# yyNoBug/VAE_segmentation

Measured on AMD Instinct MI355X. Metric: 3D train-step volumes/sec at 96^3 batch=2 (joint VAE+seg), higher is better.
Workload: dtype bf16; 1 GPU; configs[1]: 96^3 joint VAE+seg training step (joint_train), batch=2/GPU, bf16 activations + fp32 accumulate, SGD momentum 0.9, VAE frozen, HIP-graph replay; global_batch=2, parallelism=dp1, activation_recomputation=False, tail_in_graph=True, nranks=1, grad_exchange=none (1 rank)

## Files before the change

include/vaeseg.h:

```cpp
#ifndef VAESEG_H
#define VAESEG_H
#include <stddef.h>
#include <stdint.h>

#ifdef __cplusplus
extern "C" {
#endif

#define VS_VERSION 500

enum { VS_F32 = 0, VS_BF16 = 1, VS_F16 = 2, VS_F32X3 = 3  };
#ifndef VS_STAT_SLOTS
#define VS_STAT_SLOTS 4
#endif
enum { VS_OK = 0, VS_EINVAL = -1, VS_ESHAPE = -2, VS_EDTYPE = -3, VS_EWORKSPACE = -4, VS_EALIGN = -5 };

enum {
    VS_CONV_K3 = 0,
    VS_CONV_K2S2 = 1,
    VS_CONV_T2S2 = 2,
    VS_WGRAD_SLABS = 16,
    VS_CONV_UP = 3
};

enum {
    VS_PACK_ROWS_D0 = 0,
    VS_PACK_ROWS_D1_FLIP = 1,
    VS_PACK_SCATTER_D1 = 2
};

int vs_version(void);
int vs_stat_slots(void);
int vs_stat_interleaved(void);
const char* vs_strerror(int code);
int vs_get_deterministic(void);

int vs_up_supported(int cin, int cm, int co, int dtype);
int vs_up_compose_sizes(int cin, int cm, int co, size_t* out6);
int vs_up_compose(const float* w2, const float* b2, const float* w3, float* weff, void* img_fwd, void* img_bwd, int* taps_fwd, int* taps_bwd,
                  float* btab, int cin, int cm, int co, int dtype, void* stream);
int vs_up_conv_fwd(const void* x, const double* x_stats, const void* img_fwd, const int* taps_fwd, const float* btab, void* y, double* y_stats,
                   int n, int d, int h, int w, int cin, int co, int dtype, float eps, void* stream);
int vs_up_faces(const void* gy, double* G, int n, int fd, int fh, int fw, int co, int dtype, void* stream);
int vs_up_chain(const float* dweff27, const double* G, const float* w2, const float* b2, const float* w3, float* dw2, float* db2, float* dw3,
                int cin, int cm, int co, void* stream);
int vs_up_conv_bwd_data(const void* gy, const void* img_bwd, const int* taps_bwd, void* gx, const void* mask_x, const double* mask_stats,
                        double* sums, int n, int d, int h, int w, int co, int cin, int dtype, float eps, void* stream);

size_t vs_packed_weight_bytes(int rows, int c_pad, int ntaps, int dtype);
int vs_pack_weight(const float* src, void* dst, int d0, int d1, int ntaps, int c_pad, int form, int dtype, void* stream);

typedef struct vs_pack_desc {
    const float* src;
    void* dst;
    int d0, d1, ntaps, c_pad, form, dtype;
    int first_block;
    int pad_;
    long long total;
} vs_pack_desc;
int vs_pack_weight_multi(const vs_pack_desc* descs, int n_desc, int total_blocks, void* stream);

int vs_conv_gather_fwd(const void* x, const double* x_stats, const void* w_packed, const float* bias,
                       void* y, double* y_stats, int n, int d, int h, int w, int c_in, int m_out,
                       int kind, int dtype, float eps, void* stream);

int vs_conv_scatter_fwd(const void* x, const double* x_stats, const void* w_packed, const float* bias,
                        void* y, int n, int d, int h, int w, int c_in, int m_out, int dtype, float eps, void* stream);

int vs_conv_gather_bwd_data(const void* x, const void* w_packed, void* y, const void* mask_x, const double* mask_stats,
                            double* sums, int n, int d, int h, int w, int c_in, int m_out, int kind, int dtype, float eps,
                            void* stream);
int vs_conv_scatter_bwd_data(const void* x, const void* w_packed, void* y, const void* mask_x, const double* mask_stats,
                             double* sums, int n, int d, int h, int w, int c_in, int m_out, int dtype, float eps, void* stream);
int vs_conv_k3_fused_apply_supported(int n, int d, int h, int w, int c_in, int m_out, int lazy_input, int dtype);
int vs_conv_k3_bwd_data_wgrad_supported(int n, int d, int h, int w, int c_in, int m_out, int dtype);
int vs_conv_k3_bwd_data_wgrad_slabs(int n, int d, int h, int w);
int vs_conv_k3_bwd_data_wgrad(const void* g, const void* act_x, const double* act_stats, const double* act_sums, const void* w_packed, void* y,
                              const void* mask_x, const double* mask_stats, double* sums, float* slabs, int n, int d, int h, int w, int c_in,
                              int m_out, int dtype, float eps, void* stream);
int vs_conv_k3_softmax2_bwd_data(const float* prob, const float* gprob, const void* gprob_cl, const void* w_packed, void* y, const void* mask_x,
                                 const double* mask_stats, double* sums, float* slabs, double* bias_part, int n, int d, int h, int w, int dtype,
                                 float eps, float drop_p, unsigned long long drop_seed, void* stream);
typedef struct vs_config {
    int k3_small;
    int k3_tall;
    int k3_wgs_per_cu;
    int k3t_wgs_per_cu;
    int k3f_min_wgs;
    int mt_min_wgs;
    int f32_limbs;
    int g1_limbs;
    int k3x_ck;
    int k3x_toeplitz;
    int fuse_wgrad;
    int epilogue_apply;
    int chain;
    int k2s2_stream;
    int k2s8_wgs_per_cu;
    int up_wgs_per_cu;
    int up_rb;
    int wgrad_uber;
    int wgrad_mpack;
    int wgrad_swap;
    int wgrad_big;
    int wgrad_xcd;
    int k3_short_tiles;
    int wgrad_bias_fold;
    int hist_form;
    long long wgrad_wgs;
    long long wgrad_f32_tiles;
    long long wgrad_group_wgs;
    long long wgrad_big_min_voxels;
} vs_config;
int vs_config_bytes(void);
int vs_config_from_env(vs_config* c);
int vs_get_config(vs_config* out);
int vs_set_config(const vs_config* cfg);
int vs_conv_k3_bwd_data_applied_supported(int n, int d, int h, int w, int c_in, int m_out, int dtype);
int vs_conv_k3_bwd_data_applied(const void* x, const void* w_packed, void* y, const void* mask_x, const double* mask_stats, double* sums,
                                unsigned int* sync, unsigned int* fault, int n, int d, int h, int w, int c_in, int m_out, int dtype, float eps, void* stream);
int vs_conv_s2_bwd_data_applied_supported(int n, int d, int h, int w, int c_in, int m_out, int scatter, int dtype);
int vs_conv_s2_bwd_data_applied(const void* x, const void* w_packed, void* y, const void* mask_x, const double* mask_stats, double* sums, const void* add,
                                unsigned int* sync, unsigned int* fault, int n, int d, int h, int w, int c_in, int m_out, int scatter, int dtype, float eps,
                                void* stream);
typedef struct vs_chain_layer {
    const void* x;
    const double* x_stats;
    const void* w_packed;
    void* y;
    double* y_stats;
    const void* mask_x;
    const double* mask_stats;
    double* sums;
    int c_in, m_out;
    int apply;
    int reserved_;
} vs_chain_layer;
int vs_conv_k3_chain_supported(int n, int d, int h, int w, int c_max, int dtype);
long long vs_conv_k3_chain_sync_bytes(int n);
int vs_conv_k3_chain(const vs_chain_layer* layers, int n_layers, int backward, const void* add, unsigned int* sync, unsigned int* fault,
                     int n, int d, int h, int w, int dtype, float eps, void* stream);
int vs_conv_k3_f32_limbs(int d, int h, int w, int c_in);

int vs_conv_k3_bwd_data_fused_apply(const void* g, const void* act_x, const double* act_stats, const double* act_sums,
                                    const void* w_packed, void* y, const void* mask_x, const double* mask_stats, double* sums,
                                    void* dx_out, int n, int d, int h, int w, int c_in, int m_out, int dtype, float eps, void* stream);

int vs_conv_k3_softmax2_fwd(const void* x, const double* x_stats, const void* w_packed, const float* bias,
                            float* prob, int n, int d, int h, int w, int c_in, int dtype, float eps, void* stream);
int vs_conv_k3_softmax2_dropout_fwd(const void* x, const double* x_stats, const void* w_packed, const float* bias,
                                    float* prob, int n, int d, int h, int w, int c_in, int dtype, float eps, float drop_p,
                                    unsigned long long drop_seed, void* stream);
int vs_conv_k3_softmax2_cl_fwd(const void* x, const double* x_stats, const void* w_packed, const float* bias,
                               float* prob, void* prob_cl, int n, int d, int h, int w, int c_in, int dtype, float eps, float drop_p,
                               unsigned long long drop_seed, void* stream);

size_t vs_conv_wgrad_workspace_bytes(int n, int dp, int hp, int wp, int m_ch, int c_ch, int kind);
int vs_conv_wgrad(const void* p, const double* p_stats, const void* q, const double* q_stats, float* dw,
                  void* workspace, size_t workspace_bytes, int n, int dp, int hp, int wp, int m_ch, int c_ch,
                  int m_real, int c_real, int kind, int dtype, float eps, void* stream);
typedef struct vs_wgrad_desc {
    const void* p; const double* p_stats;
    const void* q; const double* q_stats;
    float* dw;
    const void* bias_g; float* db;
// ... 266 lines not shown
```

vae_segmentation_amd/modules.py:

```python
import torch
import torch.nn as nn

from . import ops

_DEFAULT_DTYPE = torch.float32


def set_default_kernel_dtype(dtype):
    global _DEFAULT_DTYPE
    if dtype not in ops.KERNEL_DTYPES:
        raise TypeError("kernel dtype must be torch.float32, torch.bfloat16 or torch.float16")
    _DEFAULT_DTYPE = dtype


def set_kernel_dtype(module, dtype):
    if dtype not in ops.KERNEL_DTYPES:
        raise TypeError("kernel dtype must be torch.float32, torch.bfloat16 or torch.float16")
    for m in module.modules():
        if hasattr(m, "kernel_dtype"):
            m.kernel_dtype = dtype
    return module


class Act:
# ... 220 lines not shown
        self.top_ch = f[5]
        flat = f[5] * self.side ** 3
        self.fc_mean = nn.Linear(flat, dim)
        self.fc_std = nn.Linear(flat, dim)
        self.fc2 = nn.Linear(dim, flat)
        self.up1 = Up(f[5], f[4], norm_type=norm_type, soft=False)
        self.up2 = Up(f[4], f[3], norm_type=norm_type, soft=False)
        self.up3 = Up(f[3], f[2], norm_type=norm_type, soft=False)
        self.up4 = Up(f[2], f[1], norm_type=norm_type, soft=False)
        self.up5 = Up(f[1], f[0], norm_type=norm_type, soft=False)
        self.out_block = nn.Conv3d(f[0], n_class, 3, padding=1)
        self.final = nn.Softmax(dim=1)
        self.n_class = n_class
        self.spatial = spatial
        self.kernel_dtype = _DEFAULT_DTYPE

    def forward(self, x, if_random=False, scale=1, mid_input=False, dropout=0.0, noise=None):
        ops._require_cuda(x)
        if not mid_input:
            if x.shape[-1] != self.spatial:
                raise ValueError("VAE built for spatial=%d got input side %d" % (self.spatial, x.shape[-1]))
            ops.stats_arena_begin(x.device)
            a = Act(ops.planar_input(x, self.kernel_dtype), None)
            a = self.in_block(a)
            if a.stats is not None:
                ops.mark_defer_apply(a.raw, self.in_block.conv[0])
            for blk in (self.down1, self.down2, self.down3, self.down4, self.down5):
                a = _run_block(blk, a)
                if blk is not self.down5 and a.stats is not None:
                    ops.mark_defer_apply(a.raw, blk.conv[1].conv[6])
            feat = ops.Materialize.apply(a.raw, a.stats, None, None)
            x_mean, x_std = ops.LinearCLPair.apply(feat, self.fc_mean.weight, self.fc_mean.bias, False,
                                                   self.fc_std.weight, self.fc_std.bias, True)
            if if_random and isinstance(noise, ops.LatentStream):
                z, _ = ops.ReparamPhilox.apply(x_mean, x_std, noise, scale)
            elif if_random:
                if noise is None:
                    noise = torch.randn(x_mean.shape, device=x_mean.device, dtype=torch.float32)
                z = ops.Reparam.apply(x_mean, x_std, noise.to(x_mean.device, torch.float32).contiguous(), scale)
            else:
                z = x_mean
        else:
            ops.stats_arena_begin(x.device)
            z = x
        h = ops.LinearToCL.apply(z, self.fc2.weight, self.fc2.bias, self.top_ch, self.side, self.kernel_dtype)
        a = Act(h, None)
        for blk in (self.up1, self.up2, self.up3, self.up4, self.up5):
            a = _dropout(_run_block(blk, a), dropout)
            if a.stats is not None:
                ops.mark_defer_apply(a.raw, blk.conv[1].conv[6])
        recon = ops.ConvK3Softmax.apply(a.raw, a.stats, self.out_block.weight, self.out_block.bias)
        if not mid_input:
            return recon, x_mean, x_std
        return recon


class Segmentation(nn.Module):

    def __init__(self, n_channels, n_class, norm_type=2, n_fmaps=[8, 16, 32, 64, 128, 256]):
        super().__init__()
        _check_n_class(n_class)
        f = list(n_fmaps)
        self.in_block = Conv(n_channels, f[0], norm_type=norm_type, soft=False)
        self.down1 = Down(f[0], f[1], norm_type=norm_type, soft=False)
        self.down2 = Down(f[1], f[2], norm_type=norm_type, soft=False)
        self.down3 = Down(f[2], f[3], norm_type=norm_type, soft=False)
        self.down4 = Down(f[3], f[4], norm_type=norm_type, soft=False)
        self.up2 = Up(f[4], f[3], norm_type=norm_type, soft=False)
        self.up3 = Up(f[3], f[2], norm_type=norm_type, soft=False)
        self.up4 = Up(f[2], f[1], norm_type=norm_type, soft=False)
        self.up5 = Up(f[1], f[0], norm_type=norm_type, soft=False)
        self.out_block = nn.Conv3d(f[0], n_class, 3, padding=1)
        self.final = nn.Softmax(dim=1)
        self.n_class = n_class
        self.kernel_dtype = _DEFAULT_DTYPE

    def forward(self, data_dict, in_key, out_key, dropout=0.0):
        x = data_dict[in_key]
        ops._require_cuda(x)
        if any(s % 16 for s in x.shape[2:]):
            raise ValueError("Segmentation needs spatial sizes that are multiples of 16, got %s" % (tuple(x.shape[2:]),))
        ops.stats_arena_begin(x.device)
        a = Act(ops.PackPlanar.apply(x, self.kernel_dtype), None)
        x1 = self.in_block(a)
        x2 = _run_block(self.down1, x1)
        x3 = _run_block(self.down2, x2)
        x4 = _run_block(self.down3, x3)
        x5 = _run_block(self.down4, x4)
        u = _dropout(_run_block(self.up2, x5), dropout)
        u = _run_block(self.up3, u)
        u = _dropout(Act(ops.Materialize.apply(u.raw, u.stats, x3.raw, x3.stats, True), None), dropout)
        tap4 = u.raw
        u = _run_block(self.up4, u)
        u = _dropout(Act(ops.Materialize.apply(u.raw, u.stats, x2.raw, x2.stats, True), None), dropout)
        if getattr(self, "ds_taps", False):
            data_dict["ds_feats"] = [u.raw, tap4]
        u = _dropout(_run_block(self.up5, u), dropout)
        if u.stats is not None:
            ops.mark_defer_apply(u.raw, self.up5.conv[1].conv[6])
        if dropout:
            data_dict[out_key] = ops.out_block_softmax(u.raw, u.stats, self.out_block.weight, self.out_block.bias,
                                                       float(dropout), ops.next_dropout_seed())
        else:
            data_dict[out_key] = ops.out_block_softmax(u.raw, u.stats, self.out_block.weight, self.out_block.bias)
        return data_dict


class DeepSupervision(nn.Module):

    def __init__(self, seg, levels=2):
        super().__init__()
        levels = int(levels)
        if levels not in (1, 2):
            raise ValueError("DeepSupervision: 1 or 2 levels (the half- and quarter-resolution skip sums), got %r" % (levels,))
        chans = [seg.up5.conv[0].in_channels, seg.up4.conv[0].in_channels][:levels]
        for c in chans:
            if c not in ops.DS_CHANNELS:
                raise NotImplementedError("DeepSupervision: the fused head reads %s feature channels, got %d" % ("/".join(map(str, ops.DS_CHANNELS)), c))
        self.heads = nn.ModuleList([nn.Conv3d(c, seg.n_class, 1) for c in chans])
        seg.ds_taps = True

    def forward(self, batch, target, scales=None, **loss_args):
        feats = batch.get("ds_feats")
        if feats is None:
            raise RuntimeError("DeepSupervision: the batch holds no 'ds_feats' — was it produced by the Segmentation this module was built on?")
        scales = [1.0] * len(self.heads) if scales is None else list(scales)
        if len(scales) != len(self.heads):
            raise ValueError("DeepSupervision: %d scales for %d levels" % (len(scales), len(self.heads)))
        return [ops.ds_head(feats[i], head.weight, head.bias, target, 2 << i, scale=scales[i], **loss_args) for i, head in enumerate(self.heads)]


class Joint(nn.Module):

    def __init__(self, models, vae_forward_scale=0.0, vae_decoder_dropout=0.0, seg_dropout=0.0):
        super().__init__()
        self.Seg = models[0]
        self.Vae = models[1]
        self.vae_forward_scale = vae_forward_scale
        self.vae_decoder_dropout = vae_decoder_dropout
        self.seg_dropout = seg_dropout

    def forward(self, data_dict, in_key, out_key, out_key_recon, dropout=False):
        with ops.arena_scope(data_dict[in_key].device):
            if dropout:
                data_dict = self.Seg(data_dict, in_key, out_key, dropout=self.seg_dropout)
                data_dict[out_key_recon], _, _ = self.Vae(data_dict[out_key], if_random=False, scale=self.vae_forward_scale,
                                                          dropout=self.vae_decoder_dropout)
            else:
                data_dict = self.Seg(data_dict, in_key, out_key)
                data_dict[out_key_recon], data_dict["mean"], data_dict["std"] = self.Vae(
                    data_dict[out_key], if_random=False, scale=self.vae_forward_scale)
        return data_dict


def _linear(x2d, fc, relu):
    return ops.LinearCL.apply(x2d.contiguous().view(x2d.shape[0], 1, 1, 1, x2d.shape[1]), fc.weight, fc.bias, relu)


class Encoder(nn.Module):

    def __init__(self, n_channels, dim, norm_type=2, n_fmaps=[8, 16, 32, 64, 128, 256], soft=False, spatial=128):
        super().__init__()
        if spatial % 32 or spatial < 64:
            raise ValueError("spatial must be a multiple of 32 and >= 64")
        f = list(n_fmaps)
        self.in_block = Conv(n_channels, f[0], norm_type=norm_type, soft=False)
        self.down1 = Down(f[0], f[1], norm_type=norm_type, soft=False)
# ... 113 lines not shown
```

vae_segmentation_amd/ops.py:

```python
import collections as _collections
import contextlib as _contextlib
import ctypes as _ctypes
import os
import weakref as _weakref

import torch

from . import _lib
from ._lib import (VS_BF16, VS_CONV_K2S2, VS_CONV_K3, VS_CONV_UP, VS_F16, VS_F32, VS_PACK_ROWS_D0, VS_PACK_ROWS_D1_FLIP,
                   VS_PACK_SCATTER_D1, _contig, _p, _require_cuda, _stream, check, lib)
from .volume import *
from .volume import signed_distance
from .volume import (PATCH_CHUNK, PATCH_LABEL_DTYPES, PATCH_MAX_CLASSES, PATCH_MAX_SOURCES, patch_gather, patch_index,
                     patch_pick)

_DT_TORCH = {VS_F32: torch.float32, VS_BF16: torch.bfloat16, VS_F16: torch.float16}
_DT_VS = {v: k for k, v in _DT_TORCH.items()}
KERNEL_DTYPES = tuple(_DT_VS)
VS_F32X3 = 3
F32X3 = "f32x3"
_DT_TORCH[VS_F32X3] = F32X3
_DT_VS[F32X3] = VS_F32X3
_F32_LIMBS = bool(lib.vs_conv_k3_f32_limbs(96, 96, 96, 8))

# ... 711 lines not shown
    _GROUP["enabled"] = bool(enabled)


def wgrad_grouping():
    return _GROUP["enabled"]


def set_wgrad_split(first=None):
    flush_wgrads()
    _GROUP["split"] = first


def drop_stale_wgrads():
    g = _GROUP
    if g["descs"] and not _PENDING["queued"]:
        return
    g["descs"], g["keep"] = [], []
    _PENDING.reset()


def _queue_desc(weight, d, dtype, nb, fl, voxels, keep):
    g = _GROUP
    if g["descs"] and g["dtype"] != dtype:
        flush_wgrads()
    g["dtype"] = dtype
    first = g["split"] is None or bool(g["split"](weight))
    g["descs"].append((d, first, nb, fl, voxels))
    g["keep"].extend(t for t in keep if t is not None)
    if not _PENDING.join():
        flush_wgrads()


def _group_submit(weight, keep, wgrad_args, bias_args, gw, gb, up_co=0):
    p, ps, q, qs, m_real, c_real, kind = wgrad_args
    n, dp, hp, wp_, m_ch = p.shape
    gw_ptr = gw if isinstance(gw, int) else gw.data_ptr()
    if kind == VS_CONV_UP:
        dp, hp, wp_, m_ch = dp // 2, hp // 2, wp_ // 2, 8 * up_co
    d = WgradDesc(p.data_ptr(), _p(ps), q.data_ptr(), _p(qs), gw_ptr, None, None, 0, 0, 0,
                  n, dp, hp, wp_, m_ch, q.shape[-1], m_real, c_real, kind, up_co)
    if bias_args is not None:
        bg = bias_args[0]
        gb_ptr = gb if isinstance(gb, int) else gb.data_ptr()
        d.bias_g, d.db, d.bias_rows, d.bias_c_ch, d.bias_c_real = bg.data_ptr(), gb_ptr, bg.numel() // bg.shape[-1], bg.shape[-1], bias_args[1]
        keep = tuple(keep) + (bg,)
    taps = 8 if kind == VS_CONV_K2S2 else 27
    nb = (p.numel() + q.numel() // q.shape[-1] * c_real) * _esize(p) + m_real * c_real * taps * 4 if kind == VS_CONV_UP else \
        (p.numel() // m_ch * m_real + q.numel() // q.shape[-1] * c_real) * _esize(p) + m_real * c_real * taps * 4
    fl = 2.0 * (q.numel() // q.shape[-1]) * taps * m_real * c_real if kind == VS_CONV_UP else 2.0 * (p.numel() // m_ch) * taps * m_real * c_real
    _queue_desc(weight, d, p.dtype, nb, fl, n * dp * hp * wp_, keep)


def pending_wgrads():
    return len(_GROUP["descs"])


def flush_wgrads(first_only=False):
    g = _GROUP
    if not g["descs"]:
        return
    now = [e for e in g["descs"] if e[1]] if first_only else g["descs"]
    later = [e for e in g["descs"] if not e[1]] if first_only else []
    g["descs"] = later
    if not now:
        return
    _issue_wgrads(now)
    if not later:
        _run_up_jobs()
        g["keep"] = []


FUSE_WGRAD = os.environ.get("VS_FUSE_WGRAD", "1") != "0"
VS_WGRAD_SLABS = 16


def _count_use(weight):
    u = getattr(weight, "_vs_use", None)
    if u is None or u[0] != _PENDING["epoch"]:
        weight._vs_use = [_PENDING["epoch"], 1]
    else:
        u[1] += 1


def _wgrad_fusable(gy, x, weight):
    if not (FUSE_WGRAD and _GROUP["enabled"] and gy.dtype != torch.float32 and gy.shape[-1] == 8 and x.shape[-1] == 8):
        return False
    if getattr(weight, "_vs_use", None) != [_PENDING["epoch"], 1] or id(weight) in _PENDING["slots"]:
        return False
    if not (weight.is_leaf and weight.grad is None and not _has_hooks(weight) and not torch.is_grad_enabled()):
        return False
    n, d, h, w, _ = gy.shape
    return bool(lib.vs_conv_k3_bwd_data_wgrad_supported(n, d, h, w, 8, 8, vs_dtype(gy)))


def _group_submit_slabs(weight, slabs, nslabs, m_real, c_real, keep, bias=None):
    gw = _grad_slot(weight, weight.shape)
    gb = None
    d = WgradDesc(slabs.data_ptr(), None, None, None, gw.data_ptr(), None, None, 0, 0, 0, nslabs, 0, 0, 0, 8, 8, m_real, c_real, VS_WGRAD_SLABS, 0)
    if bias is not None:
        gb = _grad_slot(bias[0], (m_real,))
        d.bias_g, d.db, d.bias_rows, d.bias_c_ch, d.bias_c_real = bias[1].data_ptr(), gb.data_ptr(), nslabs, m_real, m_real
    _PENDING["slots"][id(weight)] = _Slot(gw.data_ptr(), _p(gb), True)
    _queue_desc(weight, d, keep[0].dtype, float(slabs.numel() * 4), 0.0, 0, (None if bias is None else bias[1], slabs))
    return gw, gb


def _grad_slot(param, shape):
    view = getattr(param, "_vs_grad_view", None)
    if view is not None and param.grad is None:
        return view.detach()
    return torch.empty(shape, dtype=torch.float32, device=param.device)


def _has_hooks(t):
    return bool(getattr(t, "_backward_hooks", None)) or bool(getattr(t, "_post_accumulate_grad_hooks", None))


def _side_grads(weight, keep, wgrad_args, bias_args, bias=None):
    grouping = _GROUP["enabled"]
    slot = _PENDING["slots"].get(id(weight)) if grouping and weight.is_leaf else None
    if slot is not None and slot.from_slabs:
        slot = None
    if slot is not None:
        _group_submit(weight, keep, wgrad_args, bias_args if slot.gb_ptr is not None else None, slot.gw_ptr, slot.gb_ptr)
        return None, None
    gw = _grad_slot(weight, weight.shape)
    gb = None
    if bias_args is not None:
        gb = (_grad_slot(bias, (bias_args[1],)) if bias is not None else
              torch.empty(bias_args[1], dtype=torch.float32, device=keep[0].device))
    deferrable = (weight.is_leaf and weight.grad is None and not _has_hooks(weight) and not torch.is_grad_enabled()
                  and (bias is None or (bias.is_leaf and not _has_hooks(bias))))
    if grouping and deferrable:
        _PENDING["slots"][id(weight)] = _Slot(gw.data_ptr(), _p(gb), False)
        _group_submit(weight, keep, wgrad_args, bias_args, gw, gb)
        return gw, gb
    conv_wgrad(*wgrad_args, weight.shape, out_ptr=gw.data_ptr())
    if bias_args is not None:
        bias_grad(bias_args[0], bias_args[1], out_ptr=gb.data_ptr())
    return gw, gb


def _dead_bias_grad(bias, n, device):
    if bias is not None and _GROUP["enabled"]:
        if id(bias) in _PENDING["dead_biases"]:
            return None
        if _PENDING.join():
            _PENDING["dead_biases"].add(id(bias))
    view = getattr(bias, "_vs_grad_view", None) if bias is not None else None
    if view is not None and bias.grad is None:
        return view.detach()
    return _new_stats(1, (n + 1) // 2, device, width=1).view(-1).view(torch.float32)[:n]


def _conv_param_grads(weight, bias, keep, wgrad_args, bias_args, needs, live_bias=True):
    want_b = bias is not None and needs[3]
    gw = gb = None
    if needs[2]:
        gw, gb = _side_grads(weight, keep, wgrad_args, bias_args if want_b and live_bias else None, bias if live_bias else None)
    elif want_b and live_bias:
        gb = bias_grad(*bias_args)
    if want_b and not live_bias:
        gb = _dead_bias_grad(bias, bias.shape[0], weight.device)
    return gw, gb


def in_relu_bwd(g, x, xs, inplace=True):
    if xs is None:
        return g
    n, c = x.shape[0], x.shape[-1]
    voxels = x.numel() // (n * c)
    sums = _new_stats(n, c, x.device)
    dt = vs_dtype(x)
    tname = _tname(x)
    with _timed("in_relu_bwd_reduce_kernel<%s>" % tname, 2 * x.numel() * _esize(x), 4.0 * x.numel(), str(tuple(x.shape))):
        check(lib.vs_instnorm_relu_bwd_reduce(g.data_ptr(), x.data_ptr(), xs.data_ptr(), sums.data_ptr(), n, voxels, c, dt,
                                              EPS_IN, _stream()), "instnorm_relu_bwd_reduce")
    gx = g if inplace else torch.empty_like(g)
    with _timed("in_relu_bwd_apply_kernel<%s>" % tname, 3 * x.numel() * _esize(x), 6.0 * x.numel(), str(tuple(x.shape))):
        check(lib.vs_instnorm_relu_bwd_apply(g.data_ptr(), x.data_ptr(), xs.data_ptr(), sums.data_ptr(), gx.data_ptr(), n,
                                             voxels, c, dt, EPS_IN, _stream()), "instnorm_relu_bwd_apply")
    return gx


class ConvK3(torch.autograd.Function):

    @staticmethod
    def forward(ctx, x, xs, weight, bias, live_bias=False):
        _require_cuda(x, weight)
        cout, cin = weight.shape[0], weight.shape[1]
        wp = pack_weight_cached(weight, VS_PACK_ROWS_D0, x.shape[-1], k3_pack_dtype(x))
        ctx.live_bias = bool(live_bias) and bias is not None
        b_use = bias if ctx.live_bias else None
        if b_use is not None and cout < cpad(cout):
            b_use = torch.nn.functional.pad(b_use.detach().float(), (0, cpad(cout) - cout))
        y, ys = conv_gather(x, xs, wp, b_use, cpad(cout), VS_CONV_K3, True, real_channels=(cin, cout))
        ctx.save_for_backward(x, xs, weight)
        ctx.has_bias = bias is not None
        ctx.bias_ref = bias
        ctx.defer = _wants_defer(x, xs)
        if ctx.needs_input_grad[2]:
            _count_use(weight)
        ctx.mark_non_differentiable(ys)
        ctx.set_materialize_grads(False)
        return y, ys

    @staticmethod
    def backward(ctx, gy, _gys):
        x, xs, weight = ctx.saved_tensors
        if gy is None:
            return None, None, None, None, None
        gy = _contig(gy)
        cout, cin = weight.shape[0], weight.shape[1]
        gx = gw = gb = None
        lazy = _take_lazy(gy)
        if lazy is not None and not (ctx.needs_input_grad[0] and lib.vs_conv_k3_fused_apply_supported(*gy.shape, x.shape[-1], 1 if xs is not None else 0, vs_dtype(gy))):
            gy, lazy = apply_lazy(gy, lazy), None
        if ctx.needs_input_grad[0]:
            wpb = pack_weight_cached(weight, VS_PACK_ROWS_D1_FLIP, gy.shape[-1], k3_pack_dtype(gy))
            want_gb0 = ctx.has_bias and ctx.needs_input_grad[3] and ctx.live_bias
            if xs is not None and ctx.needs_input_grad[2] and not want_gb0 and _wgrad_fusable(gy, x, weight):
                gx, _, gw = _conv_bwd_data(gy, wpb, x, xs, VS_CONV_K3, real_channels=(cout, cin), defer=ctx.defer, lazy=lazy,
                                               fuse_wgrad=(weight, cout, cin))
                gb = _dead_bias_grad(ctx.bias_ref, ctx.bias_ref.shape[0], x.device) if ctx.has_bias and ctx.needs_input_grad[3] else None
                return gx, None, gw, gb, None
            if lazy is not None or xs is not None:
                gx, dx, _ = _conv_bwd_data(gy, wpb, x, xs, VS_CONV_K3, real_channels=(cout, cin), defer=ctx.defer, lazy=lazy,
                                               want_dx=ctx.needs_input_grad[2])
                if lazy is not None:
                    gy = dx
            else:
                gx, _ = conv_gather(gy, None, wpb, None, x.shape[-1], VS_CONV_K3, False, real_channels=(cout, cin))
        gw, gb = _conv_param_grads(weight, ctx.bias_ref, (gy, x, xs), (gy, None, x, xs, cout, cin, VS_CONV_K3), (gy, cout), ctx.needs_input_grad,
                                   live_bias=ctx.live_bias)
        return gx, None, gw, gb, None


CHAIN = os.environ.get("VS_CHAIN", "1") != "0"


class ChainLayer(_ctypes.Structure):
    _fields_ = [("x", _ctypes.c_void_p), ("x_stats", _ctypes.c_void_p), ("w_packed", _ctypes.c_void_p), ("y", _ctypes.c_void_p), ("y_stats", _ctypes.c_void_p),
                ("mask_x", _ctypes.c_void_p), ("mask_stats", _ctypes.c_void_p), ("sums", _ctypes.c_void_p), ("c_in", _ctypes.c_int), ("m_out", _ctypes.c_int),
                ("apply", _ctypes.c_int), ("reserved_", _ctypes.c_int)]


_CHAIN_FAULT = {}


def _chain_fault_word(device):
    key = torch.device(device)
    t = _CHAIN_FAULT.get(key)
    if t is None:
        if torch.cuda.is_current_stream_capturing():
            raise RuntimeError("the chain fault word must exist before a capture starts: run the step eagerly once (GraphedStep warms up)")
        t = _CHAIN_FAULT[key] = torch.zeros(32, dtype=torch.int32, device=key)
    return t


def chain_fault():
    for dev, t in _CHAIN_FAULT.items():
        if int(t[0].item()) != 0:
            raise _lib.VaesegError("a chain kernel on %s gave up a bounded wait (workgroups of one sample not co-resident): results invalid; set VS_CHAIN=0" % (dev,))


def device_is_shared(shared=True):
    global CHAIN, EPILOGUE_APPLY
    on = 0 if shared else 1
    set_config(chain=on, epilogue_apply=on)
    CHAIN = EPILOGUE_APPLY = not shared


def _chain_sync(n, device):
    cnt = lib.vs_conv_k3_chain_sync_bytes(n) // 8
    buf = _new_stats(1, cnt + 16, device, width=1).view(-1)
    off = ((-buf.data_ptr()) % 128) // 8
    return buf[off:off + cnt]


def chain_ok(x, xs, convs):
    if not CHAIN or len(convs) < 2 or len(convs) > 3 or x.dtype not in KERNEL_DTYPES:
        return False
    if getattr(x, "_vs_defer_apply", False):
        return False
    if any(tuple(c.weight.shape[2:]) != (3, 3, 3) for c in convs):
        return False
    n, d, h, w, c = x.shape
    cmax = max([c] + [cpad(cv.weight.shape[0]) for cv in convs])
    return bool(lib.vs_conv_k3_chain_supported(n, d, h, w, cmax, vs_dtype(x)))


class ConvK3Chain(torch.autograd.Function):

    @staticmethod
    def forward(ctx, x, xs, *params):
        _require_cuda(x)
        nl = len(params) // 2
        weights, biases = params[0::2], params[1::2]
# ... 1272 lines not shown
```

Before: 887.2 volumes/s.

## Fuse in-block norm backward apply with first-conv weight gradient

Adds a HIP kernel for the first 3x3x3 conv (1 input channel, 8 outputs). It applies the deferred instance-norm backward to the incoming gradient and accumulates the weight gradient directly against the raw planar fp32 input image, writing per-workgroup slabs. The in-block output is now marked for deferred apply, so the separate apply pass and the generic wgrad over an 8-channel padded input are skipped. The cost is a new specialised kernel with software-pipelined loads and reliance on the planar input tensor being kept alive.

```diff
diff --git a/include/vaeseg.h b/include/vaeseg.h
--- a/include/vaeseg.h
+++ b/include/vaeseg.h
@@ -81,6 +81,10 @@
 int vs_conv_k3_softmax2_bwd_data(const float* prob, const float* gprob, const void* gprob_cl, const void* w_packed, void* y, const void* mask_x,
                                  const double* mask_stats, double* sums, float* slabs, double* bias_part, int n, int d, int h, int w, int dtype,
                                  float eps, float drop_p, unsigned long long drop_seed, void* stream);
+int vs_conv_k3_in1_bwd_wgrad_supported(int n, int d, int h, int w, int m_ch, int c_real, int dtype);
+int vs_conv_k3_in1_bwd_wgrad_slabs(int n, int d, int h, int w);
+int vs_conv_k3_in1_bwd_wgrad(const void* g, const void* x, const double* x_stats, const double* sums, const void* img, int img_planar,
+                             float* slabs, int n, int d, int h, int w, int m_ch, int c_real, int dtype, float eps, void* stream);
 typedef struct vs_config {
     int k3_small;
     int k3_tall;
diff --git a/vae_segmentation_amd/csrc/inblock_bwd.hip b/vae_segmentation_amd/csrc/inblock_bwd.hip
--- /dev/null
+++ b/vae_segmentation_amd/csrc/inblock_bwd.hip
@@ -0,0 +1,228 @@
+#include "common.h"
+
+#define IB_TX 32
+#define IB_TY 16
+#define IB_TZ 4
+#define IB_PX (IB_TX + 2)
+#define IB_PY (IB_TY + 2)
+#define IB_PZ (IB_TZ + 2)
+#define IB_HALO (IB_PZ * IB_PY * IB_PX)
+#define IB_THREADS 512
+#define IB_MAX_N 64
+#define IB_MAX_WGS 512
+#define IB_SLAB_ELEMS 1728
+
+__device__ __forceinline__ void ib_fmac(float& acc, float a, float b) { asm("v_fmac_f32 %0, %1, %2" : "+v"(acc) : "v"(a), "v"(b)); }
+
+struct IBParams {
+    const void* g;
+    const void* x;
+    const double* xs;
+    const double* sums;
+    const void* img;
+    float* slabs;
+    int planar;
+    int N, D, H, W;
+    int tzn, tyn, txn, tiles;
+    double inv_count;
+    float eps;
+};
+
+template <typename T>
+__global__ __launch_bounds__(IB_THREADS) __attribute__((amdgpu_waves_per_eu(4, 4))) void inblock_bwd_kernel(const IBParams p) {
+    __shared__ float s_img[IB_HALO];
+    __shared__ float s_tab[IB_MAX_N * 8][4];
+    __shared__ float s_part[IB_THREADS / 64][4][54];
+    const int tid = threadIdx.x, lane = tid & 63, wave = tid >> 6;
+    const int cp = tid & 3, xl = (wave & 1) * 16 + ((tid >> 2) & 15), zl = wave >> 1;
+
+    for (int i = tid; i < p.N * 8; i += IB_THREADS) {
+        float m, r;
+        double sv[2];
+        stats_to_mean_rstd(p.xs, (size_t)i, (size_t)p.N * 8, p.inv_count, p.eps, m, r);
+        stat_load(p.sums, (size_t)i, (size_t)p.N * 8, sv);
+        s_tab[i][0] = m; s_tab[i][1] = r;
+        s_tab[i][2] = (float)(sv[0] * p.inv_count);
+        s_tab[i][3] = (float)(sv[1] * p.inv_count);
+    }
+
+    float acc[27][2];
+#pragma unroll
+    for (int t = 0; t < 27; ++t) acc[t][0] = acc[t][1] = 0.f;
+
+    const int per_sample = p.tzn * p.tyn * p.txn;
+    auto origin = [&](int tile, int& n, int& z0, int& y0, int& x0) {
+        n = tile / per_sample;
+        int r = tile - n * per_sample;
+        const int tz = r / (p.tyn * p.txn);
+        r -= tz * (p.tyn * p.txn);
+        const int ty = r / p.txn;
+        z0 = tz * IB_TZ; y0 = ty * IB_TY; x0 = (r - ty * p.txn) * IB_TX;
+    };
+    const unsigned int bytes = (unsigned int)((size_t)p.N * p.D * p.H * p.W * 16);
+    const i32x4 grs = make_rsrc(p.g, bytes), xrs = make_rsrc(p.x, bytes);
+    const int voff0 = ((zl * p.H) * p.W + xl) * 16 + cp * 4;
+    const int istride = p.planar ? 4 : 16;
+    const i32x4 irs = make_rsrc(p.img, (unsigned int)((size_t)p.N * p.D * p.H * p.W * istride));
+    int rq_voff = (int)0x80000000, rq_sbase = 0, rq_rows = 0;
+    auto request = [&](int tile, int yq, unsigned int (&gq)[4], unsigned int (&xq)[4]) {
+        if (yq == 0) {
+            int n, z0, y0, x0;
+            origin(tile, n, z0, y0, x0);
+            const bool live = tile < p.tiles;
+            rq_voff = (live && z0 + zl < p.D && x0 + xl < p.W) ? voff0 : (int)0x80000000;
+            rq_sbase = live ? ((((n * p.D + z0) * p.H + y0) * p.W) + x0) * 16 : 0;
+            rq_rows = live ? p.H - y0 : 0;
+        }
+        const int sbase = rq_sbase + yq * 4 * p.W * 16;
+#pragma unroll
+        for (int j = 0; j < 4; ++j) {
+            const int voff = yq * 4 + j < rq_rows ? rq_voff : (int)0x80000000;
+            gq[j] = (unsigned int)vs_raw_buffer_load_b32(grs, voff, sbase + j * p.W * 16, 0);
+            xq[j] = (unsigned int)vs_raw_buffer_load_b32(xrs, voff, sbase + j * p.W * 16, 0);
+        }
+    };
+    constexpr int NQ = IB_TY / 4;
+    constexpr int HL = (IB_HALO + IB_THREADS - 1) / IB_THREADS;
+    const int my_tiles = (p.tiles - (int)blockIdx.x + (int)gridDim.x - 1) / (int)gridDim.x;
+    const int quarters = my_tiles * NQ;
+    auto tile_of = [&](int qi) { return (int)blockIdx.x + (qi / NQ) * (int)gridDim.x; };
+    float tm[2], tr[2], ta[2], tb[2];
+    int y0 = 0;
+    bool col_ok = false;
+    auto quarter = [&](int qi, unsigned int (&gq)[4], unsigned int (&xq)[4]) {
+        const int yq = qi % NQ;
+        if (yq == 0) {
+            int n, z0, x0;
+            origin(tile_of(qi), n, z0, y0, x0);
+            unsigned int hv[HL];
+            int t0 = tid;
+            asm volatile("" : "+v"(t0));
+#pragma unroll
+            for (int k = 0; k < HL; ++k) {
+                const int i = t0 + k * IB_THREADS;
+                const int pz = i / (IB_PY * IB_PX), q = i - pz * (IB_PY * IB_PX);
+                const int py = q / IB_PX, px = q - py * IB_PX;
+                const int iz = z0 + pz - 1, iy = y0 + py - 1, ix = x0 + px - 1;
+                const bool in = i < IB_HALO && iz >= 0 && iz < p.D && iy >= 0 && iy < p.H && ix >= 0 && ix < p.W;
+                const int e = ((n * p.D + iz) * p.H + iy) * p.W + ix;
+                hv[k] = (unsigned int)vs_raw_buffer_load_b32(irs, in ? e * istride : (int)0x80000000, 0, 0);
+            }
+            __syncthreads();
+#pragma unroll
+            for (int k = 0; k < HL; ++k)
+                if (tid + k * IB_THREADS < IB_HALO)
+                    s_img[tid + k * IB_THREADS] = p.planar ? ET<T>::rnd(__uint_as_float(hv[k])) : H16<T>::lo(hv[k]);
+            __syncthreads();
+#pragma unroll
+            for (int k = 0; k < 2; ++k) {
+                const float* t = s_tab[n * 8 + 2 * cp + k];
+                tm[k] = t[0]; tr[k] = t[1]; ta[k] = t[2]; tb[k] = t[3];
+            }
+            col_ok = z0 + zl < p.D && x0 + xl < p.W;
+        }
+        float pv[4][2];
+#pragma unroll
+        for (int j = 0; j < 4; ++j) {
+            const unsigned int keep = (col_ok && y0 + yq * 4 + j < p.H) ? 0xffffffffu : 0u;
+            const float o0 = vs_in_bwd_apply1(H16<T>::lo(gq[j]), H16<T>::lo(xq[j]), tm[0], tr[0], ta[0], tb[0]);
+            const float o1 = vs_in_bwd_apply1(H16<T>::hi(gq[j]), H16<T>::hi(xq[j]), tm[1], tr[1], ta[1], tb[1]);
+            pv[j][0] = __uint_as_float(__float_as_uint(ET<T>::rnd(o0)) & keep);
+            pv[j][1] = __uint_as_float(__float_as_uint(ET<T>::rnd(o1)) & keep);
+        }
+        request(tile_of(qi + 3), (qi + 3) % NQ, gq, xq);
+        __builtin_amdgcn_sched_barrier(0);
+        const float* col = s_img + (zl * IB_PY + yq * 4) * IB_PX + xl;
+#pragma unroll
+        for (int kz = 0; kz < 3; ++kz) {
+#pragma unroll
+            for (int kx = 0; kx < 3; ++kx) {
+                float c6[6];
+#pragma unroll
+                for (int j = 0; j < 6; ++j) c6[j] = col[(kz * IB_PY + j) * IB_PX + kx];
+#pragma unroll
+                for (int j = 0; j < 4; ++j) {
+#pragma unroll
+                    for (int ky = 0; ky < 3; ++ky) {
+                        ib_fmac(acc[(kz * 3 + ky) * 3 + kx][0], pv[j][0], c6[j + ky]);
+                        ib_fmac(acc[(kz * 3 + ky) * 3 + kx][1], pv[j][1], c6[j + ky]);
+                    }
+                }
+            }
+            __builtin_amdgcn_sched_barrier(0);
+        }
+    };
+    unsigned int g0[4], x0_[4], g1[4], x1[4], g2[4], x2[4];
+    request(tile_of(0), 0, g0, x0_);
+    request(tile_of(1), 1, g1, x1);
+    request(tile_of(2), 2, g2, x2);
+#pragma unroll 1
+    for (int qi = 0; qi < quarters; qi += 3) {
+        quarter(qi, g0, x0_);
+        if (qi + 1 < quarters) quarter(qi + 1, g1, x1);
+        if (qi + 2 < quarters) quarter(qi + 2, g2, x2);
+    }
+
+#pragma unroll
+    for (int t = 0; t < 27; ++t) {
+#pragma unroll
+        for (int k = 0; k < 2; ++k) {
+            float v = acc[t][k];
+#pragma unroll
+            for (int o = 4; o < 64; o <<= 1) v += __shfl_xor(v, o, 64);
+            if (lane < 4) s_part[wave][lane][t * 2 + k] = v;
+        }
+    }
+    __syncthreads();
+    float* out = p.slabs + (size_t)blockIdx.x * IB_SLAB_ELEMS;
+    for (int o = tid; o < IB_SLAB_ELEMS; o += IB_THREADS) {
+        const int tp = o >> 6, c = (o >> 3) & 7, m = o & 7;
+        float v = 0.f;
+        if (c == 0) {
+            const int e = (26 - tp) * 2 + (m & 1);
+            for (int w = 0; w < IB_THREADS / 64; ++w) v += s_part[w][m >> 1][e];
+        }
+        out[o] = v;
+    }
+}
+
+static int ib_tiles(int n, int d, int h, int w, int* tzn, int* tyn, int* txn) {
+    *tzn = (d + IB_TZ - 1) / IB_TZ; *tyn = (h + IB_TY - 1) / IB_TY; *txn = (w + IB_TX - 1) / IB_TX;
+    const long long t = (long long)n * *tzn * *tyn * *txn;
+    return t < 2147483647ll ? (int)t : -1;
+}
+
+extern "C" int vs_conv_k3_in1_bwd_wgrad_supported(int n, int d, int h, int w, int m_ch, int c_real, int dtype) {
+    if (n <= 0 || n > IB_MAX_N || d <= 0 || h <= 0 || w <= 0) return 0;
+    if ((long long)n * d * h * w * 16 >= 2147483648ll) return 0;
+    if (m_ch != 8 || c_real != 1 || (dtype != VS_BF16 && dtype != VS_F16)) return 0;
+    int a, b, c;
+    return ib_tiles(n, d, h, w, &a, &b, &c) > 0 ? 1 : 0;
+}
+
+extern "C" int vs_conv_k3_in1_bwd_wgrad_slabs(int n, int d, int h, int w) {
+    int a, b, c;
+    const int tiles = ib_tiles(n, d, h, w, &a, &b, &c);
+    if (tiles <= 0) return 0;
+    const int rounds = (tiles + IB_MAX_WGS - 1) / IB_MAX_WGS;
+    return (tiles + rounds - 1) / rounds;
+}
+
+extern "C" int vs_conv_k3_in1_bwd_wgrad(const void* g, const void* x, const double* x_stats, const double* sums, const void* img, int img_planar,
+                                        float* slabs, int n, int d, int h, int w, int m_ch, int c_real, int dtype, float eps, void* stream) {
+    if (!g || !x || !x_stats || !sums || !img || !slabs) return VS_EINVAL;
+    if (dtype != VS_BF16 && dtype != VS_F16) return VS_EDTYPE;
+    if (!vs_conv_k3_in1_bwd_wgrad_supported(n, d, h, w, m_ch, c_real, dtype)) return VS_ESHAPE;
+    if ((((uintptr_t)g | (uintptr_t)x) & 15) || ((uintptr_t)slabs & 15)) return VS_EALIGN;
+    IBParams p;
+    p.g = g; p.x = x; p.xs = x_stats; p.sums = sums; p.img = img; p.slabs = slabs; p.planar = img_planar ? 1 : 0;
+    p.N = n; p.D = d; p.H = h; p.W = w;
+    p.tiles = ib_tiles(n, d, h, w, &p.tzn, &p.tyn, &p.txn);
+    p.inv_count = 1.0 / ((double)d * h * w);
+    p.eps = eps;
+    const int grid = vs_conv_k3_in1_bwd_wgrad_slabs(n, d, h, w);
+    if (dtype == VS_BF16) hipLaunchKernelGGL(inblock_bwd_kernel<unsigned short>, dim3(grid), dim3(IB_THREADS), 0, (hipStream_t)stream, p);
+    else hipLaunchKernelGGL(inblock_bwd_kernel<vs_half>, dim3(grid), dim3(IB_THREADS), 0, (hipStream_t)stream, p);
+    VS_CHECK_LAUNCH();
+    return VS_OK;
+}
diff --git a/vae_segmentation_amd/modules.py b/vae_segmentation_amd/modules.py
--- a/vae_segmentation_amd/modules.py
+++ b/vae_segmentation_amd/modules.py
@@ -326,7 +326,12 @@
             raise ValueError("Segmentation needs spatial sizes that are multiples of 16, got %s" % (tuple(x.shape[2:]),))
         ops.stats_arena_begin(x.device)
         a = Act(ops.PackPlanar.apply(x, self.kernel_dtype), None)
+        fuse_in = ops.FUSE_INBLOCK_BWD and x.shape[1] == 1 and self.kernel_dtype != torch.float32
+        if fuse_in:
+            a.raw._vs_planar = x
         x1 = self.in_block(a)
+        if fuse_in and x1.stats is not None:
+            ops.mark_defer_apply(x1.raw, self.in_block.conv[0])
         x2 = _run_block(self.down1, x1)
         x3 = _run_block(self.down2, x2)
         x4 = _run_block(self.down3, x3)
diff --git a/vae_segmentation_amd/ops.py b/vae_segmentation_amd/ops.py
--- a/vae_segmentation_amd/ops.py
+++ b/vae_segmentation_amd/ops.py
@@ -817,7 +817,7 @@
         u[1] += 1
 
 
-def _wgrad_fusable(gy, x, weight):
+def _wgrad_fusable(gy, x, weight, query=True):
     if not (FUSE_WGRAD and _GROUP["enabled"] and gy.dtype != torch.float32 and gy.shape[-1] == 8 and x.shape[-1] == 8):
         return False
     if getattr(weight, "_vs_use", None) != [_PENDING["epoch"], 1] or id(weight) in _PENDING["slots"]:
@@ -825,7 +825,35 @@
     if not (weight.is_leaf and weight.grad is None and not _has_hooks(weight) and not torch.is_grad_enabled()):
         return False
     n, d, h, w, _ = gy.shape
-    return bool(lib.vs_conv_k3_bwd_data_wgrad_supported(n, d, h, w, 8, 8, vs_dtype(gy)))
+    return not query or bool(lib.vs_conv_k3_bwd_data_wgrad_supported(n, d, h, w, 8, 8, vs_dtype(gy)))
+
+
+FUSE_INBLOCK_BWD = os.environ.get("VS_FUSE_INBLOCK_BWD", "1") != "0"
+
+
+def _in1_fusable(gy, x, xs, weight):
+    if not (FUSE_INBLOCK_BWD and xs is None and weight.shape[1] == 1 and tuple(weight.shape[2:]) == (3, 3, 3)):
+        return False
+    if not _wgrad_fusable(gy, x, weight, query=False):
+        return False
+    n, d, h, w, c = gy.shape
+    return bool(lib.vs_conv_k3_in1_bwd_wgrad_supported(n, d, h, w, c, weight.shape[1], vs_dtype(gy)))
+
+
+def _bwd_in1_wgrad(gy, lazy, x, planar, weight):
+    ax, axs, asums = lazy
+    n, d, h, w, c = gy.shape
+    use_planar = (planar is not None and planar.dtype == torch.float32 and planar.is_contiguous() and planar.device == gy.device
+                  and tuple(planar.shape) == (n, 1, d, h, w))
+    img = planar if use_planar else x
+    nslabs = lib.vs_conv_k3_in1_bwd_wgrad_slabs(n, d, h, w)
+    slabs = torch.empty(nslabs * 1728, dtype=torch.float32, device=gy.device)
+    vox = gy.numel() // c
+    with _timed("inblock_bwd_kernel<%s>" % _tname(gy), 2 * gy.numel() * _esize(gy) + vox * (4 if use_planar else 8 * _esize(x)), (2.0 * 27 + 6.0) * gy.numel(),
+                "apply+wgrad gy%s" % (tuple(gy.shape),)):
+        check(lib.vs_conv_k3_in1_bwd_wgrad(gy.data_ptr(), ax.data_ptr(), axs.data_ptr(), asums.data_ptr(), img.data_ptr(), 1 if use_planar else 0,
+                                           slabs.data_ptr(), n, d, h, w, c, weight.shape[1], vs_dtype(gy), EPS_IN, _stream()), "conv_k3_in1_bwd_wgrad")
+    return _group_submit_slabs(weight, slabs, nslabs, weight.shape[0], weight.shape[1], (gy, ax, axs, asums, img))[0]
 
 
 def _group_submit_slabs(weight, slabs, nslabs, m_real, c_real, keep, bias=None):
@@ -934,6 +962,7 @@
         ctx.has_bias = bias is not None
         ctx.bias_ref = bias
         ctx.defer = _wants_defer(x, xs)
+        ctx.planar = getattr(x, "_vs_planar", None)
         if ctx.needs_input_grad[2]:
             _count_use(weight)
         ctx.mark_non_differentiable(ys)
@@ -949,6 +978,12 @@
         cout, cin = weight.shape[0], weight.shape[1]
         gx = gw = gb = None
         lazy = _take_lazy(gy)
+        want_gb = ctx.has_bias and ctx.needs_input_grad[3]
+        if (lazy is not None and not ctx.needs_input_grad[0] and ctx.needs_input_grad[2] and not (want_gb and ctx.live_bias)
+                and _in1_fusable(gy, x, xs, weight)):
+            gw = _bwd_in1_wgrad(gy, lazy, x, ctx.planar, weight)
+            gb = _dead_bias_grad(ctx.bias_ref, ctx.bias_ref.shape[0], x.device) if want_gb else None
+            return None, None, gw, gb, None
         if lazy is not None and not (ctx.needs_input_grad[0] and lib.vs_conv_k3_fused_apply_supported(*gy.shape, x.shape[-1], 1 if xs is not None else 0, vs_dtype(gy))):
             gy, lazy = apply_lazy(gy, lazy), None
         if ctx.needs_input_grad[0]:
```

Result: no change. 892.3 volumes/s (median of 6 runs) (+0.6%).
